# MetaHG/mitsuba2

Measured on AMD Instinct MI355X. Metric: Msample/s, cbox 1024x1024@256spp per GPU, path integrator (max_depth=-1, rr_depth=5), higher is better.
Workload: dtype f32

## Files before the change

mitsuba2_amd/csrc/api.cpp:

```cpp
#include "../../include/mtsamd.h"
#include "bvh.h"
#include "envmap.h"
#include "kernels.h"
#include "scene_build.h"
#include "refit.h"
#include "lbvh.h"
#include "lbvh_keys.h"
#include "sah_build.h"
#include "schedule.h"
#include "spectral_upsampling.h"
#include "cie_data.h"

#include <algorithm>
#include <atomic>
#include <chrono>
#include <cmath>
#include <cstdio>
#include <cstring>
#include <cstdlib>
#include <memory>
#include <string>
#include <vector>

using namespace mtsamd;
// ... 737 lines not shown
    s->d_corner_offsets[shape] = d_offsets; s->d_corners[shape] = d_corners;
    return MTSAMD_OK;
}

static int vertex_update(mtsamd_scene *s, uint32_t shape, const float *positions, const float *normals, uint32_t flags, float *normals_out, void *stream_) {
    if (!s) return fail(MTSAMD_ERR_INVALID, "null scene");
    if (int rc = check_vertex_flags(*s, shape, normals, flags)) return rc;
    const bool recompute = (flags & MTSAMD_VERTICES_RECOMPUTE_NORMALS) != 0u;
    if (int rc = check_vertex_update(*s, shape, positions, recompute ? positions : normals)) return rc;
    HIP_TRY(hipSetDevice(s->device));
    hipStream_t stream = (hipStream_t) stream_;
    SceneGeometry &g = s->geometry;
    if (g.flat) return flat_vertex_update(s, shape, positions, normals, recompute, normals_out, stream);
    const uint32_t nv = 3u * g.shape_vertices[shape], off = g.shapes[shape].first_prim, n_faces = g.shape_faces[shape];
    const int32_t em = g.shapes[shape].emitter;
    const RefitView rv = refit_view(s);
    if (recompute)
        if (int rc = corner_table(s, shape, stream)) return rc;
    HIP_TRY(hipMemcpyAsync(s->d_stage_pos, positions, nv * sizeof(float), hipMemcpyDefault, stream));
    if (normals) HIP_TRY(hipMemcpyAsync(s->d_stage_nrm, normals, nv * sizeof(float), hipMemcpyDefault, stream));
    HIP_TRY(hipMemsetAsync(s->d_refit_flag, 0, sizeof(uint32_t), stream));
    HIP_TRY(launch_refit_check(rv, s->d_stage_pos, nv, off, n_faces, em >= 0 ? s->d_stage_area : nullptr, s->d_refit_flag, stream));
    uint32_t flag = 0;
    std::vector<float> pmf(em >= 0 ? n_faces : 0), cdf(pmf.size());
    HIP_TRY(hipMemcpyAsync(&flag, s->d_refit_flag, sizeof(flag), hipMemcpyDeviceToHost, stream));
    if (em >= 0 && n_faces) HIP_TRY(hipMemcpyAsync(pmf.data(), s->d_stage_area, n_faces * sizeof(float), hipMemcpyDeviceToHost, stream));
    HIP_TRY(hipStreamSynchronize(stream));
    if (flag) return fail(MTSAMD_ERR_INVALID, "shape %u: a vertex has a non-finite coordinate", shape);
    DevEmitter e{};
    if (em >= 0) {
        e = s->emitters[em];
        if (int rc = area_distribution(pmf.data(), n_faces, cdf.data(), e)) return rc;
    }
    if (recompute) {
        HIP_TRY(launch_refit_normals(rv, s->d_stage_pos, off, n_faces, g.shape_vertices[shape], s->d_corner_offsets[shape], s->d_corners[shape],
                                     s->d_face_recs, s->d_stage_nrm, stream));
        if (normals_out) HIP_TRY(hipMemcpyAsync(normals_out, s->d_stage_nrm, nv * sizeof(float), hipMemcpyDefault, stream));
    }
    HIP_TRY(launch_refit_gather(rv, s->d_stage_pos, normals || recompute ? s->d_stage_nrm : nullptr, off, n_faces, stream));
    for (size_t h = 0; h + 1 < s->class_start.size(); ++h)
        HIP_TRY(launch_refit_boxes(rv, s->class_start[h], s->class_start[h + 1] - s->class_start[h], h == 0, stream));
    HIP_TRY(hipMemcpyAsync(s->bvh.bbox, s->d_boxes + 6 * (size_t) s->refit_root, 6 * sizeof(float), hipMemcpyDeviceToHost, stream));
    HIP_TRY(hipStreamSynchronize(stream));
    RefitGrid grid{};
    scene_grid(s->bvh.bbox, &grid.extent, s->bvh.q_lo, s->bvh.q_step);
    for (int k = 0; k < 3; ++k) {
        grid.glo[k] = (double) s->bvh.q_lo[k]; grid.gstep[k] = (double) s->bvh.q_step[k];
        s->view.q_lo[k] = s->bvh.q_lo[k]; s->view.q_step[k] = s->bvh.q_step[k]; s->view.q_inv_step[k] = 1.0f / s->bvh.q_step[k];
    }
    if (em >= 0) s->emitters[em] = e;
    set_scene_bounds(*s);
    HIP_TRY(launch_refit_emit(rv, grid, stream));
    if (em >= 0 && n_faces) {
        HIP_TRY(hipMemcpyAsync(s->d_area_pmf + off, pmf.data(), n_faces * sizeof(float), hipMemcpyHostToDevice, stream));
        HIP_TRY(hipMemcpyAsync(s->d_area_cdf + off, cdf.data(), n_faces * sizeof(float), hipMemcpyHostToDevice, stream));
// ... 1526 lines not shown
```

mitsuba2_amd/csrc/kernels.hip:

```cpp
#include "kernels.h"

namespace mtsamd {

constexpr int kBlock = 256;
static_assert(kBlock == 64 * (int) kShadeWaves, "k_shade LDS sizing (kernels.h)");

struct PathState {
    f3 o, d; float mint, maxt;
    f3 thr; float bs_pdf;
    f3 res; float eta;
    Pcg32 rng;
    uint32_t ordinal, depth, flags;
};

template <bool NT = false>
MTS_DEV void load_state(const PoolView &p, size_t i, PathState &s) {
    float4 a = ld_stream<NT>(p.ray_o + i), b = ld_stream<NT>(p.ray_d + i), c = ld_stream<NT>(p.thr + i), e = ld_stream<NT>(p.res + i);
    uint4 r = ld_stream<NT>(p.rng + i); uint2 m = ld_stream<NT>(p.misc + i);
    s.o = mk3(a.x, a.y, a.z); s.mint = a.w;
    s.d = mk3(b.x, b.y, b.z); s.maxt = b.w;
    s.thr = mk3(c.x, c.y, c.z); s.bs_pdf = c.w;
    s.res = mk3(e.x, e.y, e.z); s.eta = e.w;
    s.rng.state = (uint64_t) r.x | ((uint64_t) r.y << 32);
    s.rng.inc = (uint64_t) r.z | ((uint64_t) r.w << 32);
// ... 31 lines not shown
    static constexpr bool kSamples = false;
    template <int DEFER, bool GENERAL, bool NEST> MTS_DEV void begin(const PathState &s) { }
    MTS_DEV void emitted(float ew, int32_t emitter, f3 le) { }
    MTS_DEV void escaped(const SceneView &sv, const PathState &s, const DevEmitter &e, float ew, f3 le) { }
    MTS_DEV void roulette(f3 thr, float hm, float rq, bool free) { }
    MTS_DEV void surface(const SurfaceInteraction &si, const DevBsdf &bsdf, f3 refl, uint32_t texel, f2 tw1, f3 thr) { }
    MTS_DEV bool emitter_sample(const SceneView &sv, const DevBsdf &bsdf, f3 refl, const NeeTerms &t) { return false; }
    MTS_DEV void unoccluded(const SceneView &sv, const SurfaceInteraction &si, f3 thr, const NeeTerms &t) { }
    MTS_DEV void bsdf_sampled(const SceneView &sv, const SurfaceInteraction &si, const DevBsdf &bsdf, f3 refl, f3 thr, const BsdfSample &bs, f3 weight, float s1, f2 s2) { }
};

template <bool NEST, bool FLAT> struct BsdfTable;
template <bool FLAT> struct BsdfTable<false, FLAT> {
    const Geo<FLAT> &geo;
    MTS_DEV BsdfTable(const Geo<FLAT> &g, const f2 &) : geo(g) { }
    MTS_DEV DevBsdf operator()(uint32_t i) const { return geo.bsdf(i); }
};
template <bool FLAT> struct BsdfTable<true, FLAT> {
    const Geo<FLAT> &geo; const f2 &uv;
    MTS_DEV BsdfTable(const Geo<FLAT> &g, const f2 &t) : geo(g), uv(t) { }
    MTS_DEV DevBsdf operator()(uint32_t i) const { DevBsdf rec = geo.bsdf(i); resolve_textured(geo.sv, rec, uv); return rec; }
};

template <bool FLAT, int DEFER = 0, bool GENERAL = false, bool NEST = false, class Probe = NoProbe>
MTS_DEV bool bounce_step(const RenderParams &P, const LdsView &lds, PathState &s, Counters &c, Probe &&probe = Probe{}, Deferred *df = nullptr) {
    using Pr = std::remove_reference_t<Probe>;
    static_assert(!NEST || (GENERAL && DEFER == 0), "blendbsdf / mask run the general fused step");
    const SceneView &sv = P.sv;
    probe.template begin<DEFER, GENERAL, NEST>(s);
    const Geo<FLAT> geo{ sv, lds };
    Hit hit;
    ++c.closest; ++c.segments;
    bool found;
    if (DEFER) df->pending = false;
    if (DEFER == 1) { hit = df->hit; found = df->found; }
    else found = traverse<FLAT, false>(sv, lds, s.o, s.d, s.mint, s.maxt, hit, c.tri_tests,
                                       FLAT && __ballot(s.depth != 1u) == 0ull);
    if (s.depth == 1u) s.flags = found ? 1u : 0u;

    SurfaceInteraction si;
    if (found) {
        fill_si(geo, s.d, hit.prim, hit.u, hit.v, si);
        int32_t emitter = si.shape_rec.emitter;
        if (emitter >= 0) {
            const DevEmitter e = geo.emitter((uint32_t) emitter);
            float ew = 1.0f;
            if (s.depth > 1u) {
// ... 96 lines not shown

    const float s1 = pcg_next_f32(s.rng);
    f2 s2; s2.x = pcg_next_f32(s.rng); s2.y = pcg_next_f32(s.rng);
    f3 wo, weight; float pdf;
    if (GENERAL) {
        BsdfSample bs;
        surface_bsdf_sample<NEST>(bsdf, ni, refl, BsdfTable<NEST, FLAT>(geo, si.uv), child_refl, si.wi, s1, s2, bs, weight);
        wo = bs.wo; pdf = bs.pdf;
        s.eta *= bs.eta;
        s.flags = bs.delta ? (s.flags | kFlagDelta) : (s.flags & ~kFlagDelta);
        if (Pr::kSamples) probe.bsdf_sampled(sv, si, bsdf, refl, s.thr, bs, weight, s1, s2);
    } else {
        diffuse_sample(refl, wi_b, s2, wo, pdf, weight);
        if (flip) wo.z = -wo.z;
    }
    s.thr = mk3(s.thr.x * weight.x, s.thr.y * weight.y, s.thr.z * weight.z);
    if (!(s.thr.x != 0.0f || s.thr.y != 0.0f || s.thr.z != 0.0f)) return false;
    s.o = si.p;
    s.d = to_world(si.sh, wo);
    s.mint = (1.0f + hmax_abs(si.p)) * kRayEpsilon;
    s.maxt = __builtin_inff();
    s.bs_pdf = pdf;
    s.depth += 1u;
    return true;
}

template <bool GENERAL = true>
MTS_DEV void generate_path(const RenderParams &P, uint64_t ordinal, uint32_t lp, uint32_t j, PathState &s, float2 *pos_out = nullptr) {
    const uint32_t w = (uint32_t) P.crop_w;
    const uint32_t lr = lp / w, px = lp - lr * w;
    const uint32_t py = (uint32_t) row_to_global(P.rows, (int32_t) lr);
    const uint64_t index = ((uint64_t) py * w + px) * (uint64_t) P.spp + j;
    seed_sample(s.rng, index, P.base_seed);
    float jx = pcg_next_f32(s.rng), jy = pcg_next_f32(s.rng);
    float psx = ((float) px + (float) P.crop_x) + jx, psy = ((float) py + (float) P.crop_y) + jy;
    f2 ap; ap.x = ap.y = 0.5f;
    if (GENERAL && P.cam.aperture_radius > 0.0f) { ap.x = pcg_next_f32(s.rng); ap.y = pcg_next_f32(s.rng); }
    (void) pcg_next_f32(s.rng);
    float ax = (psx - (float) P.crop_x) / (float) P.crop_w, ay = (psy - (float) P.crop_y) / (float) P.crop_h;
    camera_ray<GENERAL>(P.cam, ax, ay, ap, s.o, s.d, s.mint, s.maxt);
    s.thr = mk3(1.0f, 1.0f, 1.0f); s.bs_pdf = 0.0f;
    s.res = mk3(0.0f, 0.0f, 0.0f); s.eta = 1.0f;
    s.ordinal = P.plane_pixels ? j * P.plane_pixels + (lp - P.plane_pix0) : (uint32_t) (ordinal - P.first_ordinal);
    s.depth = 1u; s.flags = 0u;
    if (P.out_pos) P.out_pos[s.ordinal] = make_float2(psx, psy);
    if (pos_out) *pos_out = make_float2(psx, psy);
// ... 415 lines not shown
        surface_bsdf_sample<NEST, kWav>(bsdf, ni, [&](uint32_t i) { return geo.bsdf(i); }, chan_of, si.wi, s1, s2, bs, w);
        wo = bs.wo; pdf = bs.pdf;
        s.eta *= bs.eta;
        s.flags = bs.delta ? (s.flags | kFlagDelta) : (s.flags & ~kFlagDelta);
        if constexpr (kWatch) probe.bsdf_sampled(sv, si, bsdf, refl, s.thr, bs, w);
#pragma unroll
        for (int k = 0; k < kWav; ++k) { s.thr.v[k] = s.thr.v[k] * w[k]; nz = nz || s.thr.v[k] != 0.0f; }
    } else {
        if (si.wi.z > 0.0f) {
            wo = square_to_cosine_hemisphere(s2);
            pdf = kInvPi * wo.z;
            ok = pdf > 0.0f;
        }
#pragma unroll
        for (int k = 0; k < kWav; ++k) { s.thr.v[k] = s.thr.v[k] * (ok ? refl.v[k] : 0.0f); nz = nz || s.thr.v[k] != 0.0f; }
    }
    if (!nz) return false;
    s.o = si.p;
    s.d = to_world(si.sh, wo);
    s.mint = (1.0f + hmax_abs(si.p)) * kRayEpsilon;
    s.maxt = __builtin_inff();
    s.bs_pdf = pdf;
    s.depth += 1u;
    return true;
}

MTS_DEV void generate_path_spectral(const RenderParams &P, uint64_t ordinal, uint32_t lp, uint32_t j, PathStateS &s, float2 *pos_out = nullptr) {
    const uint32_t w = (uint32_t) P.crop_w;
    const uint32_t lr = lp / w, px = lp - lr * w;
    const uint32_t py = (uint32_t) row_to_global(P.rows, (int32_t) lr);
    const uint64_t index = ((uint64_t) py * w + px) * (uint64_t) P.spp + j;
    seed_sample(s.rng, index, P.base_seed);
    float jx = pcg_next_f32(s.rng), jy = pcg_next_f32(s.rng);
    float psx = ((float) px + (float) P.crop_x) + jx, psy = ((float) py + (float) P.crop_y) + jy;
    f2 ap; ap.x = ap.y = 0.5f;
    if (P.cam.aperture_radius > 0.0f) { ap.x = pcg_next_f32(s.rng); ap.y = pcg_next_f32(s.rng); }
    s.xi = pcg_next_f32(s.rng);
    wavelengths_from_sample(s.xi, s.wav);
    float ax = (psx - (float) P.crop_x) / (float) P.crop_w, ay = (psy - (float) P.crop_y) / (float) P.crop_h;
    camera_ray(P.cam, ax, ay, ap, s.o, s.d, s.mint, s.maxt);
#pragma unroll
    for (int k = 0; k < kWav; ++k) { s.thr.v[k] = 1.0f; s.res.v[k] = 0.0f; }
    s.bs_pdf = 0.0f; s.eta = 1.0f;
    s.ordinal = P.plane_pixels ? j * P.plane_pixels + (lp - P.plane_pix0) : (uint32_t) (ordinal - P.first_ordinal);
    s.depth = 1u; s.flags = 0u;
    if (P.out_pos) P.out_pos[s.ordinal] = make_float2(psx, psy);
// ... 332 lines not shown
MTS_DEV void start_path(const RenderParams &P, uint64_t ordinal, uint32_t lp, uint32_t j, PathState &s) { generate_path(P, ordinal, lp, j, s); }
MTS_DEV void start_path(const RenderParams &P, uint64_t ordinal, uint32_t lp, uint32_t j, PathStateS &s) { generate_path_spectral(P, ordinal, lp, j, s); }

#ifndef MTS_SHADE_WAVES_MIN
#define MTS_SHADE_WAVES_MIN 4
#endif
#ifndef MTS_SHADE_WAVES_MIN_RGB_DIFFUSE
#define MTS_SHADE_WAVES_MIN_RGB_DIFFUSE 5
#endif
template <typename State, bool GENERAL> struct ShadeWaves { static constexpr int kMin = MTS_SHADE_WAVES_MIN; };
template <> struct ShadeWaves<PathState, false> { static constexpr int kMin = MTS_SHADE_WAVES_MIN_RGB_DIFFUSE; };
template <typename State> struct ShadowRing {
    static constexpr bool kSlotInNee = false;
    static constexpr uint32_t kFloat4 = kShadowRing * 13u / 4u;
    float4 *o, *d, *nee; uint32_t *slot;
};
template <> struct ShadowRing<PathState> {
    static constexpr bool kSlotInNee = true;
    static constexpr uint32_t kFloat4 = kShadowRing * 3u;
    float4 *o, *d, *nee; uint32_t *slot;
};
static_assert(ShadowRing<PathState>::kFloat4 * 16u == 48u * kShadowRing && ShadowRing<PathStateS>::kFloat4 * 16u == 52u * kShadowRing,
              "ring sizes of shadow_ring_bytes()");

template <typename State, bool GENERAL>
MTS_DEV void drain_shadow_ring(const RenderParams &P, const LdsView &lds, const ShadowRing<State> &q, uint32_t head, uint32_t count,
                               size_t base, Counters &c) {
    __builtin_amdgcn_fence(__ATOMIC_SEQ_CST, "workgroup");
    const uint32_t lane = lane_id();
    if (lane < count) {
        const uint32_t k = (head + lane) & (kShadowRing - 1u);
        const float4 o = q.o[k], d = q.d[k];
        Hit h;
        if (!traverse<true, true>(P.sv, lds, mk3(o.x, o.y, o.z), mk3(d.x, d.y, d.z), o.w, d.w, h, c.tri_tests)) {
            const float4 e = q.nee[k];
            const size_t slot = base + (ShadowRing<State>::kSlotInNee ? __float_as_uint(e.w) : q.slot[k]);
            float4 r = P.out.res[slot];
            r.x += e.x; r.y += e.y; r.z += e.z;
            if (!ShadowRing<State>::kSlotInNee) r.w += e.w;
            P.out.res[slot] = r;
        }
    }
}

#ifndef MTS_NT_STREAMS
#define MTS_NT_STREAMS 3
#endif
#ifndef MTS_PRIMARY_SHADOW
#define MTS_PRIMARY_SHADOW 1
#endif
#ifndef MTS_SURV_ORDER
#define MTS_SURV_ORDER 1
#endif
template <typename State, bool GENERAL, bool FLAT, bool INLINE = false>
__global__ __launch_bounds__(kBlock) __attribute__((amdgpu_waves_per_eu(FLAT ? MTS_BOUNCE_WAVES : ShadeWaves<State, GENERAL>::kMin, FLAT ? MTS_BOUNCE_WAVES : 8)))
void k_shade(const RenderParams P) {
    static_assert(FLAT || !INLINE, "the in-kernel shadow queue is for LDS-resident scenes");
// ... 98 lines not shown
            if (s.flags & kFlagZombie) {
                finish_path(P, s);
            } else {
                depth0 = s.depth;
                if (!FLAT) {
                    const float4 h = ld_stream<kNT>(P.in.hit + i);
                    df.hit.t = h.x; df.hit.prim = __float_as_uint(h.y); df.hit.u = h.z; df.hit.v = h.w;
                    df.found = df.hit.prim != kNoPrim;
                }
                alive = step_deferred<GENERAL, FLAT>(P, lds, s, c, df);
                if (!alive) {
                    if (df.pending) { s.flags |= kFlagZombie; alive = true; zombie_now = true; }
                    else finish_path(P, s);
                }
            }
        }
        if (INLINE && MTS_FLAT_CULL && MTS_PRIMARY_SHADOW && P.sv.n_clusters > 1u && __ballot(depth0 != 1u && (i0 + lane < n_in)) == 0ull) {
            if (df.pending) {
                if (!traverse_flat_clustered_any(P.sv, lds, df.so, df.sd, df.smint, df.smaxt, c.tri_tests)) add_nee(s, df.nee);
                df.pending = false;
                if (zombie_now) { s.flags &= ~kFlagZombie; finish_path(P, s); alive = false; }
            }
        }
        const uint64_t m = __ballot(alive), ms = __ballot(alive && df.pending);
        if (alive) {
            const uint32_t slot = n_out + mask_rank(m);
            const size_t oidx = (FLAT && gw > 4u) ? ((size_t) wave + 4u * (slot / P.seg_cap)) * P.seg_cap + slot % P.seg_cap : base + slot;
            store_state<kNT>(P.out, oidx, s);
            if (df.pending) {
                if (INLINE) {
                    const uint32_t k = (q_head + q_count + mask_rank(ms)) & (kShadowRing - 1u);
                    ring.o[k] = make_float4(df.so.x, df.so.y, df.so.z, df.smint);
                    ring.d[k] = make_float4(df.sd.x, df.sd.y, df.sd.z, df.smaxt);
                    const uint32_t rslot = (uint32_t) (oidx - base);
                    if (ShadowRing<State>::kSlotInNee) {
                        ring.nee[k] = make_float4(df.nee[0], df.nee[1], df.nee[2], __uint_as_float(rslot));
                    } else {
                        ring.nee[k] = make_float4(df.nee[0], df.nee[1], df.nee[2], df.nee[3]);
                        ring.slot[k] = rslot;
                    }
                } else {
                    const size_t q = base + n_sh + mask_rank(ms);
                    st_stream<kNT>(P.out.sh_o + q, make_float4(df.so.x, df.so.y, df.so.z, df.smint));
                    st_stream<kNT>(P.out.sh_d + q, make_float4(df.sd.x, df.sd.y, df.sd.z, df.smaxt));
                    st_stream<kNT>(P.out.nee + q, make_float4(df.nee[0], df.nee[1], df.nee[2], df.nee[3]));
                    st_stream<kNT>(P.out.sh_slot + q, slot);
                }
            }
        }
        n_out += (uint32_t) __popcll(m);
        n_sh += (uint32_t) __popcll(ms);
        if (INLINE) {
            q_count += (uint32_t) __popcll(ms);
            if (q_count >= 64u) {
                drain_shadow_ring<State, GENERAL>(P, lds, ring, q_head, 64u, base, c);
                q_head = (q_head + 64u) & (kShadowRing - 1u); q_count -= 64u;
            }
        }
    }
    if (INLINE && q_count > 0u) drain_shadow_ring<State, GENERAL>(P, lds, ring, q_head, q_count, base, c);

    const uint32_t n_surv = n_out;
    uint64_t cursor = P.cursor[wave];
    const uint64_t end = P.cursor_end[wave];
    while (n_out < P.target && cursor < end) {
        uint64_t left = end - cursor;
        uint32_t n_new = min(64u, P.target - n_out);
        if ((uint64_t) n_new > left) n_new = (uint32_t) left;
        if (lane < n_new) {
            State s;
            uint64_t ordinal; uint32_t lp, sj;
            cursor_sample(P, wave, cursor + lane, ordinal, lp, sj);
// ... 5 lines not shown

    uint32_t tot[4] = { c.closest, c.any, c.segments, c.tri_tests };
#pragma unroll
    for (int k = 0; k < 4; ++k)
        for (int off = 32; off > 0; off >>= 1) tot[k] += __shfl_xor(tot[k], off);
    if (FLAT && gw > 4u) {
        for (uint32_t q = lane; q < gw / 4u; q += 64u) {
            const uint32_t w2 = wave + 4u * q, lo = q * P.seg_cap;
            if (w2 < wave_last) P.count_out[w2] = n_out > lo ? min(n_out - lo, P.seg_cap) : 0u;
        }
    }
    if (lane == 0) {
        if (!(FLAT && gw > 4u)) P.count_out[wave] = n_out;
        if (FLAT && !(gw > 4u)) P.count_out[P.n_waves + wave] = n_surv;
        if (!INLINE) P.count_shadow[wave] = n_sh;
        P.cursor[wave] = cursor;
        uint64_t *ws = P.wave_stats + 4u * (size_t) wave;
        ws[0] += tot[0]; ws[1] += tot[1]; ws[2] += tot[2];
        if (FLAT) ws[3] += tot[3];
    }
}

constexpr uint32_t kFinishMaxPer = 1024u, kFinishLdsDepth = 8u;
template <bool GENERAL, bool FLAT>
MTS_DEV bool step_fused(const RenderParams &P, const LdsView &lds, PathState &s, Counters &c) { return bounce_step<FLAT, 0, GENERAL>(P, lds, s, c); }
template <bool GENERAL, bool FLAT>
MTS_DEV bool step_fused(const RenderParams &P, const LdsView &lds, PathStateS &s, Counters &c) { return bounce_step_spectral<FLAT, false, GENERAL>(P, lds, s, c); }
template <bool GENERAL, bool FLAT>
MTS_DEV bool step_fused(const RenderParams &P, const LdsView &lds, PathStateT &s, Counters &c) { return bounce_step_spectral<FLAT, 0, GENERAL, false, NoProbeS, true>(P, lds, s, c); }

template <typename State, bool GENERAL, bool FLAT>
__global__ __launch_bounds__(64) void k_finish(const RenderParams P, uint32_t per) {
    extern __shared__ float4 smem[];
    __shared__ uint32_t s_pre[kFinishMaxPer + 1];
    const uint32_t lane = threadIdx.x, w0 = blockIdx.x * per;
    const uint32_t n_w = min(per, P.n_waves - min(P.n_waves, w0));
    {
        const uint32_t run = (n_w + 63u) / 64u;
        uint32_t local = 0u;
        for (uint32_t i = 0; i < run; ++i) { const uint32_t k = lane * run + i; if (k < n_w) local += P.count_in[w0 + k]; }
        uint32_t incl = local;
        for (uint32_t off = 1u; off < 64u; off <<= 1) { const uint32_t v = __shfl_up(incl, off); if (lane >= off) incl += v; }
        uint32_t sum = incl - local;
        if (lane == 0u) s_pre[0] = 0u;
        for (uint32_t i = 0; i < run; ++i) { const uint32_t k = lane * run + i; if (k < n_w) { sum += P.count_in[w0 + k]; s_pre[k + 1u] = sum; } }
    }
    __syncthreads();
    const uint32_t total = s_pre[n_w];
    if (total == 0u) return;
    for (uint32_t k = lane; k < n_w; k += 64u) P.count_out[w0 + k] = 0u;
    LdsView lds = {};
// ... 51 lines not shown
        lds.stack_lds_depth = min(P.sv.stack_depth, kFinishLdsDepth);
        lds.spill = reinterpret_cast<StackEntry *>(P.trace_spill) + (size_t) blockIdx.x * (P.sv.stack_depth - lds.stack_lds_depth) * 64u + lane;
        lds.spill_stride = 64u;
    }
    Counters c = { 0u, 0u, 0u, 0u };
    State s;
    bool busy = false;
    while (true) {
        const uint64_t m = __ballot(!busy);
        if (m != 0ull && cursor < end) {
            const uint64_t v = cursor + mask_rank(m);
            if (!busy && v < end) {
                uint64_t ordinal; uint32_t lp, sj;
                cursor_sample(P, wave, v, ordinal, lp, sj);
                start_path(P, ordinal, lp, sj, s);
                busy = true;
            }
            cursor += (uint64_t) __popcll(m);
        }
        if (__ballot(busy) == 0ull) {
            if (cursor >= end) break;
            continue;
        }
        if (busy && !step_fused<GENERAL, FLAT>(P, lds, s, c)) { finish_path(P, s); busy = false; }
    }
    uint32_t tot[4] = { c.closest, c.any, c.segments, c.tri_tests };
#pragma unroll
    for (int k = 0; k < 4; ++k)
        for (int off = 32; off > 0; off >>= 1) tot[k] += __shfl_xor(tot[k], off);
    if (lane == 0u) {
        P.cursor[wave] = end;
        uint64_t *ws = P.wave_stats + 4u * (size_t) wave;
        ws[0] += tot[0]; ws[1] += tot[1]; ws[2] += tot[2]; ws[3] += tot[3];
    }
}

template <typename S> struct VariantState { using type = S; };
template <typename F> static void with_variant(const RenderParams &p, F &&f) {
    if (p.spectral && p.sv.n_spectra) f(VariantState<PathStateT>{}, std::true_type{});
    else if (p.spectral && p.sv.general) f(VariantState<PathStateS>{}, std::true_type{});
    else if (p.spectral) f(VariantState<PathStateS>{}, std::false_type{});
    else if (p.sv.general) f(VariantState<PathState>{}, std::true_type{});
    else f(VariantState<PathState>{}, std::false_type{});
}
template <typename F> static void with_flag(bool v, F &&f) { if (v) f(std::true_type{}); else f(std::false_type{}); }
#define MTS_VARIANT(st, general) typename decltype(st)::type, decltype(general)::value

// ... 2543 lines not shown
```

mitsuba2_amd/csrc/scene_build.cpp:

```cpp
#include "scene_build.h"
#include "vertex_normals.h"

#include <algorithm>
#include <cmath>
#include <cstdarg>
#include <cstdio>
#include <cstring>
#include <limits>
#include <string>

namespace mtsamd {

namespace { thread_local std::string g_last_error; }

int fail(int code, const char *fmt, ...) {
    char buf[1024];
    va_list ap; va_start(ap, fmt); vsnprintf(buf, sizeof(buf), fmt, ap); va_end(ap);
    g_last_error = buf;
    return code;
}
const char *last_error() { return g_last_error.c_str(); }

int srgb_colour(const Rgb2Spec &model, const float rgb[3], float coeff[3], float *mean, float *jac9) {
    if (!srgb_in_range(rgb))
// ... 317 lines not shown
            return fail(MTSAMD_ERR_INVALID, "texture %u: image must be at least 2x2 pixels in size", t);
    }
    return check_texture_bindings(in);
}

int validate(Input &in, int32_t &environment) {
    const mtsamd_scene_desc *desc = &in.desc;
    if (int rc = check_spectrum_bindings(in)) return rc;
    if (desc->mesh_count > 0 && !desc->meshes) return fail(MTSAMD_ERR_INVALID, "scene has no shapes");
    if (desc->mesh_count > 0 && (desc->bsdf_count == 0 || !desc->bsdfs)) return fail(MTSAMD_ERR_INVALID, "scene has no BSDFs");
    std::vector<int32_t> emitter_shape(desc->emitter_count, -1);
    if (int rc = validate_meshes(in, emitter_shape)) return rc;
    if (int rc = validate_emitters(desc, emitter_shape, environment)) return rc;
    if (int rc = validate_bsdfs(in)) return rc;
    if (in.total >= (1ull << 27)) return fail(MTSAMD_ERR_UNSUPPORTED, "too many primitives (%llu)", (unsigned long long) in.total);
    return MTSAMD_OK;
}

int area_emitter(const mtsamd_emitter_desc &ed, uint32_t shape, uint32_t off, uint32_t face_count, HostScene &hs, DevEmitter &e) {
    for (uint32_t f = 0; f < face_count; ++f) hs.area_pmf[off + f] = triangle_area(&hs.tri_pos[9 * (size_t) (off + f)]);
    std::memset(&e, 0, sizeof(e));
    e.r = ed.radiance[0]; e.g = ed.radiance[1]; e.b = ed.radiance[2];
    e.shape = shape; e.first_prim = off; e.n_prims = face_count;
    return area_distribution(&hs.area_pmf[off], face_count, &hs.area_cdf[off], e);
}

int flatten_meshes(const Input &in, HostScene &hs) {
    const mtsamd_scene_desc *desc = &in.desc;
    const uint64_t total = in.total;
    hs.tri_pos.assign(9 * total, 0.0f); hs.tri_nrm.assign(in.any_nrm ? 9 * total : 0, 0.0f); hs.tri_uv.assign(in.any_uv ? 6 * total : 0, 0.0f);
    hs.prim_shape.assign(total, 0u);
    hs.shapes.assign(desc->mesh_count, DevShape{});
    hs.area_pmf.assign(total, 0.0f); hs.area_cdf.assign(total, 0.0f);
    SceneGeometry &g = hs.state.geometry;
    g.faces.assign(3 * total, 0u); g.shape_vertices.assign(desc->mesh_count, 0u); g.shape_faces.assign(desc->mesh_count, 0u);
    uint32_t off = 0;
    for (uint32_t i = 0; i < desc->mesh_count; ++i) {
        const mtsamd_mesh_desc &m = desc->meshes[i];
        DevShape &sh = hs.shapes[i];
        sh.bsdf = m.bsdf; sh.emitter = m.emitter; sh.first_prim = off;
        sh.flags = (m.normals ? kShapeHasNormals : 0u) | (m.texcoords ? kShapeHasUV : 0u);
        g.shape_vertices[i] = m.vertex_count; g.shape_faces[i] = m.face_count;
        for (uint32_t f = 0; f < m.face_count; ++f) {
            uint32_t gp = off + f;
            hs.prim_shape[gp] = i;
            for (int j = 0; j < 3; ++j) {
// ... 627 lines not shown

int area_distribution(const float *areas, uint32_t face_count, float *cdf, DevEmitter &e) {
    double sum = 0.0; uint32_t lo = 0xffffffffu, hi = 0xffffffffu;
    for (uint32_t f = 0; f < face_count; ++f) {
        sum += (double) areas[f];
        cdf[f] = (float) sum;
        if (areas[f] > 0.0f) { if (lo == 0xffffffffu) lo = f; hi = f; }
    }
    if (lo == 0xffffffffu) return fail(MTSAMD_ERR_INVALID, "DiscreteDistribution: no probability mass found!");
    e.area_sum = (float) sum; e.area_norm = (float) (1.0 / sum);
    e.valid_lo = lo; e.valid_hi = hi;
    return MTSAMD_OK;
}

void set_scene_bounds(SceneState &st) {
    float centre[3], radius;
    bounding_sphere(st.bvh.bbox, centre, &radius);
    if (st.environment >= 0) {
        DevEmitter &e = st.emitters[st.environment];
        e.cx = centre[0]; e.cy = centre[1]; e.cz = centre[2]; e.radius = radius;
    }
    for (DevEmitter &e : st.emitters)
        if (e.pad0 == kEmitterDirectional) e.radius = radius;
}

int check_vertex_update(const SceneState &st, uint32_t shape, const float *positions, const float *normals) {
    const SceneGeometry &g = st.geometry;
    if (shape >= g.shapes.size()) return fail(MTSAMD_ERR_INVALID, "invalid shape index %u (the scene has %u shapes)", shape, (uint32_t) g.shapes.size());
    if (!positions) return fail(MTSAMD_ERR_INVALID, "shape %u: null vertex positions", shape);
    const bool has = (g.shapes[shape].flags & kShapeHasNormals) != 0u;
    if (has && !normals) return fail(MTSAMD_ERR_INVALID, "shape %u was created with vertex normals: new normals are required with new positions", shape);
    if (!has && normals) return fail(MTSAMD_ERR_INVALID, "shape %u was created without vertex normals: none can be set", shape);
    return MTSAMD_OK;
}

int check_vertex_flags(const SceneState &st, uint32_t shape, const float *normals, uint32_t flags) {
    const SceneGeometry &g = st.geometry;
    const uint32_t known = MTSAMD_VERTICES_RECOMPUTE_NORMALS | MTSAMD_VERTICES_REBUILD_ACCEL | ((flags & MTSAMD_VERTICES_REBUILD_ACCEL) ? MTSAMD_VERTICES_ACCEL_SAH : 0u);
    if (flags & ~known) return fail(MTSAMD_ERR_INVALID, "unknown vertex update flags 0x%x", flags & ~(uint32_t) MTSAMD_VERTICES_RECOMPUTE_NORMALS);
    if (!(flags & MTSAMD_VERTICES_RECOMPUTE_NORMALS)) return MTSAMD_OK;
    if (shape >= g.shapes.size()) return fail(MTSAMD_ERR_INVALID, "invalid shape index %u (the scene has %u shapes)", shape, (uint32_t) g.shapes.size());
    if (normals) return fail(MTSAMD_ERR_INVALID, "shape %u: MTSAMD_VERTICES_RECOMPUTE_NORMALS computes the normals: none can be passed with it", shape);
    if (!(g.shapes[shape].flags & kShapeHasNormals))
        return fail(MTSAMD_ERR_INVALID, "shape %u was created without vertex normals: storing new normals in such a mesh is not implemented", shape);
    return MTSAMD_OK;
}
// ... 30 lines not shown
        for (int j = 0; j < 3; ++j) {
            const uint32_t vi = g.faces[3 * (size_t) (off + f) + j];
            for (int k = 0; k < 3; ++k) {
                tri_pos[9 * (size_t) f + 3 * j + k] = positions[3 * (size_t) vi + k];
                if (normals) tri_nrm[9 * (size_t) f + 3 * j + k] = normals[3 * (size_t) vi + k];
            }
        }
}

int set_vertex_positions(SceneState &st, const BuildOptions &opt, uint32_t shape, const float *positions, const float *normals,
                         std::vector<float> &tri_pos, std::vector<float> &tri_nrm, std::vector<float> &area_pmf, std::vector<float> &area_cdf, FlatRecords &flat) {
    if (int rc = check_vertex_update(st, shape, positions, normals)) return rc;
    const SceneGeometry &g = st.geometry;
    if (int rc = check_finite(shape, positions, 3 * (size_t) g.shape_vertices[shape])) return rc;
    const uint32_t off = g.shapes[shape].first_prim, n = g.shape_faces[shape];
    std::vector<float> pos(9 * (size_t) n), nrm(normals ? 9 * (size_t) n : 0), pmf(n), cdf(n);
    gather_shape(g, shape, positions, normals, pos.data(), nrm.data());
    const int32_t em = g.shapes[shape].emitter;
    DevEmitter e{};
    if (em >= 0) {
        e = st.emitters[em];
        for (uint32_t f = 0; f < n; ++f) pmf[f] = triangle_area(&pos[9 * (size_t) f]);
        if (int rc = area_distribution(pmf.data(), n, cdf.data(), e)) return rc;
    }
    std::copy(pos.begin(), pos.end(), tri_pos.begin() + 9 * (size_t) off);
    if (normals) std::copy(nrm.begin(), nrm.end(), tri_nrm.begin() + 9 * (size_t) off);
    if (em >= 0) {
        st.emitters[em] = e;
        std::copy(pmf.begin(), pmf.end(), area_pmf.begin() + off); std::copy(cdf.begin(), cdf.end(), area_cdf.begin() + off);
    }
    refit_bvh(tri_pos.data(), st.bvh);
    set_scene_bounds(st);
    const bool was_flat = flat.flat;
    build_flat_records(opt, st, tri_pos, flat);
    if (flat.flat != was_flat) return fail(MTSAMD_ERR_DEVICE, "vertex update: the scene changed its kind");
    return MTSAMD_OK;
}

}
```

mitsuba2_amd/csrc/scene_build.h:

```cpp
#pragma once
#include "../../include/mtsamd.h"
#include "bvh.h"
#include "envmap.h"
#include "kernels.h"
#include "spectral_upsampling.h"

#include <cstdint>
#include <vector>

namespace mtsamd {

int fail(int code, const char *fmt, ...);
const char *last_error();

inline float rgb_mean(const float c[3]) { return (c[0] + c[1] + c[2]) * (1.0f / 3.0f); }
inline float plastic_lobe_weight(float d_mean, float s_mean) { return s_mean / (d_mean + s_mean); }
inline bool srgb_in_range(const float c[3]) { return !(c[0] < 0 || c[1] < 0 || c[2] < 0 || c[0] > 1 || c[1] > 1 || c[2] > 1); }
int srgb_colour(const Rgb2Spec &model, const float rgb[3], float coeff[3], float *mean, float *jac9);
void srgb_d65_colour(const Rgb2Spec &model, const float rgb[3], DevEmitter &e);
float bitmap_luminance_mean(const float *rgb, size_t n_texels);
bool invert_linear3(const float to_world[16], float inv[9]);
void bounding_sphere(const float bbox[6], float centre[3], float *radius);

int check_spectrum(const mtsamd_spectrum_desc &sp, uint32_t index, double *integral);
// ... 47 lines not shown

struct HostScene : FlatRecords {
    SceneState state;
    std::vector<float> tri_pos, tri_nrm, tri_uv;
    std::vector<uint32_t> prim_shape;
    std::vector<DevShape> shapes;
    std::vector<float> area_pmf, area_cdf;
    std::vector<DevBsdf> bsdf_block;
    uint32_t n_spectra = 0;
    std::vector<const float *> tex_src;
    std::vector<std::vector<float>> tex_coeffs;
    bool has_envmap = false;
    EnvmapHost env;
    DevEnvmap dev_env{};
};

int build_host_scene(const mtsamd_scene_desc *desc, const mtsamd_spectrum_desc *spectra, uint32_t n_spectra,
                     const mtsamd_spectrum_binding *bindings, uint32_t n_bindings, const BuildOptions &options, HostScene &hs,
                     const mtsamd_texture_binding *tex_bindings = nullptr, uint32_t n_tex_bindings = 0);

float triangle_area(const float *tri_pos9);
int area_distribution(const float *areas, uint32_t face_count, float *cdf, DevEmitter &e);
void set_scene_bounds(SceneState &st);
void build_flat_records(const BuildOptions &opt, const SceneState &st, const std::vector<float> &tri_pos, FlatRecords &out);
int check_vertex_update(const SceneState &st, uint32_t shape, const float *positions, const float *normals);
int check_finite(uint32_t shape, const float *positions, size_t n_floats);
void gather_shape(const SceneGeometry &g, uint32_t shape, const float *positions, const float *normals, float *tri_pos, float *tri_nrm);
void compute_vertex_normals(uint32_t vertex_count, const float *positions, uint32_t face_count, const uint32_t *faces, float *normals_out);
void build_corner_table(uint32_t vertex_count, uint32_t face_count, const uint32_t *faces, std::vector<uint32_t> &offsets, std::vector<uint32_t> &corners);
int check_vertex_flags(const SceneState &st, uint32_t shape, const float *normals, uint32_t flags);
int set_vertex_positions(SceneState &st, const BuildOptions &opt, uint32_t shape, const float *positions, const float *normals,
                         std::vector<float> &tri_pos, std::vector<float> &tri_nrm, std::vector<float> &area_pmf, std::vector<float> &area_cdf, FlatRecords &flat);

bool bsdf_param_fields(const DevBsdf &b, int32_t kind, int32_t comp, float DevBsdf::*&f0, float DevBsdf::*&f1);
int build_tangent_records(const SceneState &st, const float *bsdf_tangents, float h, std::vector<DevBsdf> &plus, std::vector<DevBsdf> &minus,
                          std::vector<float> &inv_2h);
int build_reverse_slots(const SceneState &st, const uint8_t *wanted, float h, std::vector<ReverseSlot> &slots, std::vector<uint32_t> &range);
int set_bsdf_reflectance(SceneState &st, uint32_t bsdf, const float *rgb);
int set_bsdf_param(SceneState &st, uint32_t bsdf, int32_t kind, const float *value3);
int set_emitter_radiance(SceneState &st, uint32_t emitter, const float *rgb);
bool texture_feeds_lobe_weight(const SceneState &st, uint32_t texture);
void set_texture_texels(SceneState &st, uint32_t texture, float *rgb, std::vector<float> &coeffs, std::vector<uint32_t> &changed_bsdfs);
int set_envmap_texels(SceneState &st, const float *rgb, EnvmapHost &eh);

}
```

Measured before the change: 3965.

## Elide closest-hit traversal for paths fated to terminate when ray misses emitters

After a bounce, peeks the next Russian-roulette random number and depth limit to decide whether the path will terminate at the next vertex. If so, and the continuation ray cannot reach any area emitter's padded bounding box, the closest-hit traversal is skipped and the path finishes immediately, since only emitter hits would add radiance. Emitter boxes are computed at build and refit time, and pending shadow rays for such finished paths are routed through the shadow ring with a final-entry flag that writes the result directly. This adds per-bounce box tests and extra bookkeeping, and it relies on the peeked RNG value matching what the path would consume at the next step.

New measurement: 4158 (median of 6 runs). 4.9% higher.

```diff
diff --git a/mitsuba2_amd/csrc/api.cpp b/mitsuba2_amd/csrc/api.cpp
--- a/mitsuba2_amd/csrc/api.cpp
+++ b/mitsuba2_amd/csrc/api.cpp
@@ -783,15 +783,17 @@
     HIP_TRY(hipMemsetAsync(s->d_refit_flag, 0, sizeof(uint32_t), stream));
     HIP_TRY(launch_refit_check(rv, s->d_stage_pos, nv, off, n_faces, em >= 0 ? s->d_stage_area : nullptr, s->d_refit_flag, stream));
     uint32_t flag = 0;
-    std::vector<float> pmf(em >= 0 ? n_faces : 0), cdf(pmf.size());
+    std::vector<float> pmf(em >= 0 ? n_faces : 0), cdf(pmf.size()), em_pos(em >= 0 ? nv : 0);
     HIP_TRY(hipMemcpyAsync(&flag, s->d_refit_flag, sizeof(flag), hipMemcpyDeviceToHost, stream));
     if (em >= 0 && n_faces) HIP_TRY(hipMemcpyAsync(pmf.data(), s->d_stage_area, n_faces * sizeof(float), hipMemcpyDeviceToHost, stream));
+    if (em >= 0 && nv) HIP_TRY(hipMemcpyAsync(em_pos.data(), s->d_stage_pos, nv * sizeof(float), hipMemcpyDeviceToHost, stream));
     HIP_TRY(hipStreamSynchronize(stream));
     if (flag) return fail(MTSAMD_ERR_INVALID, "shape %u: a vertex has a non-finite coordinate", shape);
     DevEmitter e{};
     if (em >= 0) {
         e = s->emitters[em];
         if (int rc = area_distribution(pmf.data(), n_faces, cdf.data(), e)) return rc;
+        emitter_exact_box(em_pos.data(), nv / 3u, e);
     }
     if (recompute) {
         HIP_TRY(launch_refit_normals(rv, s->d_stage_pos, off, n_faces, g.shape_vertices[shape], s->d_corner_offsets[shape], s->d_corners[shape],
diff --git a/mitsuba2_amd/csrc/fated.h b/mitsuba2_amd/csrc/fated.h
--- /dev/null
+++ b/mitsuba2_amd/csrc/fated.h
@@ -0,0 +1,54 @@
+#pragma once
+#include "flat_cull.h"
+
+#ifndef MTS_FATED_ELIDE
+#define MTS_FATED_ELIDE 1
+#endif
+#ifndef MTS_FATED_ELIDE_SPECTRAL
+#define MTS_FATED_ELIDE_SPECTRAL 0
+#endif
+#ifndef MTS_FATED_STATS
+#define MTS_FATED_STATS 0
+#endif
+
+namespace mtsamd {
+
+constexpr uint32_t kFatedMaxBoxes = 4u;
+constexpr int kFatedBox = 0, kFatedExact = 8, kFatedList = 15;
+
+inline void fated_encode(const float lo[3], const float hi[3], float pad, float *aux) {
+    float plo[3], phi[3];
+    for (int a = 0; a < 3; ++a) { plo[a] = lo[a] - pad; phi[a] = hi[a] + pad; }
+    float4 r0, r1;
+    cull_encode<1>(plo, phi, 0u, 0u, r0, r1);
+    aux[kFatedBox + 0] = r0.x; aux[kFatedBox + 1] = r0.y; aux[kFatedBox + 2] = r0.z; aux[kFatedBox + 3] = 0.0f;
+    aux[kFatedBox + 4] = r1.x; aux[kFatedBox + 5] = r1.y; aux[kFatedBox + 6] = r1.z; aux[kFatedBox + 7] = 0.0f;
+}
+inline void fated_invalidate(float *aux) {
+    for (int a = 0; a < 3; ++a) { aux[kFatedBox + a] = 0.0f; aux[kFatedBox + 4 + a] = INFINITY; }
+    aux[kFatedBox + 3] = aux[kFatedBox + 7] = 0.0f;
+}
+
+__host__ __device__ inline float fated_peek_f32(uint64_t state) {
+    const uint32_t xs = (uint32_t) (((state >> 18u) ^ state) >> 27u);
+    const uint32_t rot = (uint32_t) (state >> 59u);
+    const uint32_t u = (xs >> rot) | (xs << ((~rot + 1u) & 31));
+    return __builtin_bit_cast(float, (u >> 9) | 0x3f800000u) - 1.0f;
+}
+
+__host__ __device__ inline bool fated_decide(uint32_t depth, int32_t max_depth, int32_t rr_depth, float hm, float eta, uint64_t rng_state) {
+    bool fated = depth >= (uint32_t) max_depth;
+    if ((int32_t) depth > rr_depth) {
+        const float q = fminf(hm * (eta * eta), 0.95f);
+        fated = fated || !(fated_peek_f32(rng_state) < q);
+    }
+    return fated;
+}
+
+__host__ __device__ inline bool fated_reach(const CullLean &q, const float *aux, float mint, float maxt) {
+    const float4 r0 = make_float4(aux[kFatedBox + 0], aux[kFatedBox + 1], aux[kFatedBox + 2], 0.0f);
+    const float4 r1 = make_float4(aux[kFatedBox + 4], aux[kFatedBox + 5], aux[kFatedBox + 6], 0.0f);
+    return cull_reach(q, r0, r1, mint, maxt);
+}
+
+}
diff --git a/mitsuba2_amd/csrc/kernels.hip b/mitsuba2_amd/csrc/kernels.hip
--- a/mitsuba2_amd/csrc/kernels.hip
+++ b/mitsuba2_amd/csrc/kernels.hip
@@ -1,4 +1,5 @@
 #include "kernels.h"
+#include "fated.h"
 
 namespace mtsamd {
 
@@ -77,7 +78,25 @@
     MTS_DEV DevBsdf operator()(uint32_t i) const { DevBsdf rec = geo.bsdf(i); resolve_textured(geo.sv, rec, uv); return rec; }
 };
 
-template <bool FLAT, int DEFER = 0, bool GENERAL = false, bool NEST = false, class Probe = NoProbe>
+template <bool FLAT>
+MTS_DEV bool fated_elide(const RenderParams &P, const LdsView &lds, const f3 &o, const f3 &d, float mint, float maxt, float hm, float eta, uint32_t depth,
+                         uint64_t rng_state, Counters &c) {
+    const SceneView &sv = P.sv;
+    if (sv.env_emitter >= 0 || sv.n_emitters == 0u) return false;
+    const DevEmitter *em = FLAT ? lds.emitters : sv.emitters;
+    const uint32_t list = __float_as_uint(em[0].aux[kFatedList]);
+    if (list == 0u) return false;
+    if (!fated_decide(depth, P.max_depth, P.rr_depth, hm, eta, rng_state)) return false;
+    const CullLean q = cull_ray<CullLean>(o.x, o.y, o.z, d.x, d.y, d.z);
+    for (uint32_t l = list; l != 0u; l >>= 8)
+        if (fated_reach(q, em[(l & 0xffu) - 1u].aux, mint, maxt)) return false;
+    if (!MTS_FATED_STATS) ++c.closest;
+    ++c.segments;
+    if (FLAT && !(MTS_CULL_STATS & 1)) c.tri_tests += sv.n_prims;
+    return true;
+}
+
+template <bool FLAT, int DEFER = 0, bool GENERAL = false, bool NEST = false, class Probe = NoProbe, bool ELIDE = true>
 MTS_DEV bool bounce_step(const RenderParams &P, const LdsView &lds, PathState &s, Counters &c, Probe &&probe = Probe{}, Deferred *df = nullptr) {
     using Pr = std::remove_reference_t<Probe>;
     static_assert(!NEST || (GENERAL && DEFER == 0), "blendbsdf / mask run the general fused step");
@@ -220,6 +239,8 @@
     s.maxt = __builtin_inff();
     s.bs_pdf = pdf;
     s.depth += 1u;
+    if constexpr (MTS_FATED_ELIDE && ELIDE && std::is_same_v<Pr, NoProbe>)
+        if (fated_elide<FLAT>(P, lds, s.o, s.d, s.mint, s.maxt, fmaxf(fmaxf(s.thr.x, s.thr.y), s.thr.z), s.eta, s.depth, s.rng.state, c)) return false;
     return true;
 }
 
@@ -681,6 +702,9 @@
     s.maxt = __builtin_inff();
     s.bs_pdf = pdf;
     s.depth += 1u;
+    if constexpr (MTS_FATED_ELIDE && MTS_FATED_ELIDE_SPECTRAL && !kWatch)
+        if (fated_elide<FLAT>(P, lds, s.o, s.d, s.mint, s.maxt, fmaxf(fmaxf(s.thr.v[0], s.thr.v[1]), fmaxf(s.thr.v[2], s.thr.v[3])), s.eta, s.depth,
+                              s.rng.state, c)) return false;
     return true;
 }
 
@@ -1059,6 +1083,19 @@
 };
 static_assert(ShadowRing<PathState>::kFloat4 * 16u == 48u * kShadowRing && ShadowRing<PathStateS>::kFloat4 * 16u == 52u * kShadowRing,
               "ring sizes of shadow_ring_bytes()");
+constexpr uint32_t kRingFinal = 0x80000000u;
+template <typename State> constexpr bool kRingFinishes = MTS_FATED_ELIDE != 0 && ShadowRing<State>::kSlotInNee;
+MTS_DEV bool finish_ring_entry(const RenderParams &P, const float4 &e, bool occluded) {
+    const uint32_t w = __float_as_uint(e.w);
+    if (!(w & kRingFinal)) return false;
+    PathState t;
+    t.ordinal = w & ~kRingFinal;
+    const float4 r = P.out_rgba[t.ordinal];
+    t.res = occluded ? mk3(r.x, r.y, r.z) : mk3(r.x + e.x, r.y + e.y, r.z + e.z);
+    t.flags = r.w != 0.0f ? 1u : 0u;
+    store_result(P, t);
+    return true;
+}
 
 template <typename State, bool GENERAL>
 MTS_DEV void drain_shadow_ring(const RenderParams &P, const LdsView &lds, const ShadowRing<State> &q, uint32_t head, uint32_t count,
@@ -1069,7 +1106,10 @@
         const uint32_t k = (head + lane) & (kShadowRing - 1u);
         const float4 o = q.o[k], d = q.d[k];
         Hit h;
-        if (!traverse<true, true>(P.sv, lds, mk3(o.x, o.y, o.z), mk3(d.x, d.y, d.z), o.w, d.w, h, c.tri_tests)) {
+        const bool occluded = traverse<true, true>(P.sv, lds, mk3(o.x, o.y, o.z), mk3(d.x, d.y, d.z), o.w, d.w, h, c.tri_tests);
+        bool finished = false;
+        if constexpr (kRingFinishes<State>) finished = finish_ring_entry(P, q.nee[k], occluded);
+        if (!finished && !occluded) {
             const float4 e = q.nee[k];
             const size_t slot = base + (ShadowRing<State>::kSlotInNee ? __float_as_uint(e.w) : q.slot[k]);
             float4 r = P.out.res[slot];
@@ -1214,7 +1254,14 @@
                 if (zombie_now) { s.flags &= ~kFlagZombie; finish_path(P, s); alive = false; }
             }
         }
-        const uint64_t m = __ballot(alive), ms = __ballot(alive && df.pending);
+        bool final_now = false;
+        if constexpr (INLINE && kRingFinishes<State>) {
+            if (zombie_now && df.pending) {
+                P.out_rgba[s.ordinal] = make_float4(s.res.x, s.res.y, s.res.z, (s.flags & 1u) ? 1.0f : 0.0f);
+                alive = false; final_now = true;
+            }
+        }
+        const uint64_t m = __ballot(alive), ms = __ballot((alive || final_now) && df.pending);
         if (alive) {
             const uint32_t slot = n_out + mask_rank(m);
             const size_t oidx = (FLAT && gw > 4u) ? ((size_t) wave + 4u * (slot / P.seg_cap)) * P.seg_cap + slot % P.seg_cap : base + slot;
@@ -1240,6 +1287,14 @@
                 }
             }
         }
+        if constexpr (INLINE && kRingFinishes<State>) {
+            if (final_now) {
+                const uint32_t k = (q_head + q_count + mask_rank(ms)) & (kShadowRing - 1u);
+                ring.o[k] = make_float4(df.so.x, df.so.y, df.so.z, df.smint);
+                ring.d[k] = make_float4(df.sd.x, df.sd.y, df.sd.z, df.smaxt);
+                ring.nee[k] = make_float4(df.nee[0], df.nee[1], df.nee[2], __uint_as_float(s.ordinal | kRingFinal));
+            }
+        }
         n_out += (uint32_t) __popcll(m);
         n_sh += (uint32_t) __popcll(ms);
         if (INLINE) {
@@ -1291,11 +1346,11 @@
 }
 
 constexpr uint32_t kFinishMaxPer = 1024u, kFinishLdsDepth = 8u;
-template <bool GENERAL, bool FLAT>
-MTS_DEV bool step_fused(const RenderParams &P, const LdsView &lds, PathState &s, Counters &c) { return bounce_step<FLAT, 0, GENERAL>(P, lds, s, c); }
-template <bool GENERAL, bool FLAT>
+template <bool GENERAL, bool FLAT, bool ELIDE = true>
+MTS_DEV bool step_fused(const RenderParams &P, const LdsView &lds, PathState &s, Counters &c) { return bounce_step<FLAT, 0, GENERAL, false, NoProbe, ELIDE>(P, lds, s, c); }
+template <bool GENERAL, bool FLAT, bool ELIDE = true>
 MTS_DEV bool step_fused(const RenderParams &P, const LdsView &lds, PathStateS &s, Counters &c) { return bounce_step_spectral<FLAT, false, GENERAL>(P, lds, s, c); }
-template <bool GENERAL, bool FLAT>
+template <bool GENERAL, bool FLAT, bool ELIDE = true>
 MTS_DEV bool step_fused(const RenderParams &P, const LdsView &lds, PathStateT &s, Counters &c) { return bounce_step_spectral<FLAT, 0, GENERAL, false, NoProbeS, true>(P, lds, s, c); }
 
 template <typename State, bool GENERAL, bool FLAT>
@@ -1393,7 +1448,7 @@
             if (cursor >= end) break;
             continue;
         }
-        if (busy && !step_fused<GENERAL, FLAT>(P, lds, s, c)) { finish_path(P, s); busy = false; }
+        if (busy && !step_fused<GENERAL, FLAT, FLAT || GENERAL>(P, lds, s, c)) { finish_path(P, s); busy = false; }
     }
     uint32_t tot[4] = { c.closest, c.any, c.segments, c.tri_tests };
 #pragma unroll
diff --git a/mitsuba2_amd/csrc/scene_build.cpp b/mitsuba2_amd/csrc/scene_build.cpp
--- a/mitsuba2_amd/csrc/scene_build.cpp
+++ b/mitsuba2_amd/csrc/scene_build.cpp
@@ -1,4 +1,5 @@
 #include "scene_build.h"
+#include "fated.h"
 #include "vertex_normals.h"
 
 #include <algorithm>
@@ -363,6 +364,7 @@
     std::memset(&e, 0, sizeof(e));
     e.r = ed.radiance[0]; e.g = ed.radiance[1]; e.b = ed.radiance[2];
     e.shape = shape; e.first_prim = off; e.n_prims = face_count;
+    emitter_exact_box(&hs.tri_pos[9 * (size_t) off], 3 * (size_t) face_count, e);
     return area_distribution(&hs.area_pmf[off], face_count, &hs.area_cdf[off], e);
 }
 
@@ -1036,6 +1038,36 @@
     }
     for (DevEmitter &e : st.emitters)
         if (e.pad0 == kEmitterDirectional) e.radius = radius;
+    set_emitter_boxes(st);
+}
+
+void emitter_exact_box(const float *xyz, size_t n_points, DevEmitter &e) {
+    float lo[3] = { 3e38f, 3e38f, 3e38f }, hi[3] = { -3e38f, -3e38f, -3e38f };
+    for (size_t i = 0; i < n_points; ++i)
+        for (int a = 0; a < 3; ++a) { lo[a] = std::min(lo[a], xyz[3 * i + a]); hi[a] = std::max(hi[a], xyz[3 * i + a]); }
+    for (int a = 0; a < 3; ++a) { e.aux[kFatedExact + a] = lo[a]; e.aux[kFatedExact + 3 + a] = hi[a]; }
+}
+
+void set_emitter_boxes(SceneState &st) {
+    if (st.emitters.empty()) return;
+    float ext = 0.0f;
+    for (int k = 0; k < 6; ++k) ext = std::max(ext, std::fabs(st.bvh.bbox[k]));
+    const float pad = 1e-4f * std::max(ext, 1e-3f);
+    uint32_t list = 0u, n = 0u;
+    bool off = st.environment >= 0;
+    for (size_t i = 0; i < st.emitters.size(); ++i) {
+        DevEmitter &e = st.emitters[i];
+        if (e.pad0 != 0u) continue;
+        const float lo[3] = { e.aux[kFatedExact], e.aux[kFatedExact + 1], e.aux[kFatedExact + 2] };
+        const float hi[3] = { e.aux[kFatedExact + 3], e.aux[kFatedExact + 4], e.aux[kFatedExact + 5] };
+        if (std::isfinite(pad)) fated_encode(lo, hi, pad, e.aux);
+        else fated_invalidate(e.aux);
+        if (n < kFatedMaxBoxes && i < 255u) list |= (uint32_t) (i + 1u) << (8u * n);
+        else off = true;
+        ++n;
+    }
+    if (off || n == 0u) list = 0u;
+    std::memcpy(&st.emitters[0].aux[kFatedList], &list, 4);
 }
 
 int check_vertex_update(const SceneState &st, uint32_t shape, const float *positions, const float *normals) {
@@ -1112,6 +1144,7 @@
         e = st.emitters[em];
         for (uint32_t f = 0; f < n; ++f) pmf[f] = triangle_area(&pos[9 * (size_t) f]);
         if (int rc = area_distribution(pmf.data(), n, cdf.data(), e)) return rc;
+        emitter_exact_box(pos.data(), 3 * (size_t) n, e);
     }
     std::copy(pos.begin(), pos.end(), tri_pos.begin() + 9 * (size_t) off);
     if (normals) std::copy(nrm.begin(), nrm.end(), tri_nrm.begin() + 9 * (size_t) off);
diff --git a/mitsuba2_amd/csrc/scene_build.h b/mitsuba2_amd/csrc/scene_build.h
--- a/mitsuba2_amd/csrc/scene_build.h
+++ b/mitsuba2_amd/csrc/scene_build.h
@@ -93,6 +93,8 @@
 float triangle_area(const float *tri_pos9);
 int area_distribution(const float *areas, uint32_t face_count, float *cdf, DevEmitter &e);
 void set_scene_bounds(SceneState &st);
+void emitter_exact_box(const float *xyz, size_t n_points, DevEmitter &e);
+void set_emitter_boxes(SceneState &st);
 void build_flat_records(const BuildOptions &opt, const SceneState &st, const std::vector<float> &tri_pos, FlatRecords &out);
 int check_vertex_update(const SceneState &st, uint32_t shape, const float *positions, const float *normals);
 int check_finite(uint32_t shape, const float *positions, size_t n_floats);
```
